# SarthakYadav/leaf-pytorch

Hardware: AMD Instinct MI355X
Metric: LEAF frames/s (40 filt, 16 kHz, 1 s clips) (higher is better)
Workload: dtype f32

## Files before the change

leaf_pytorch_amd/csrc/leaf_fft_wg.hpp:

```cpp
#pragma once
#include <type_traits>
#include "leaf_fft.hpp"
#include "leaf_inst.hpp"
#include "leaf_wg_queue.hpp"

namespace {

constexpr int kWgRingFloat2 = 1032;
constexpr int kWgFwdBins = 1152;
constexpr int kWgRingFwdFloat2 = kWgFwdBins + 8;

typedef float v2f __attribute__((ext_vector_type(2)));
constexpr int kWgScrStride = 68;
constexpr int kWgScrFloats = 32 * kWgScrStride;

__device__ __forceinline__ unsigned lds_addr(const void* p) {
    return (unsigned)(size_t)(__attribute__((address_space(3))) const char*)p;
}
template <int OFF>
__device__ __forceinline__ void lds_rd8(v2f& dst, unsigned addr) {
    asm volatile("ds_read_b64 %0, %1 offset:%2" : "=v"(dst) : "v"(addr), "i"(OFF));
}
template <int N>
__device__ __forceinline__ void lds_wait8(v2f (&a)[8]) {
    asm volatile("s_waitcnt lgkmcnt(%8)"
                 : "+v"(a[0]), "+v"(a[1]), "+v"(a[2]), "+v"(a[3]), "+v"(a[4]), "+v"(a[5]), "+v"(a[6]), "+v"(a[7])
                 : "i"(N));
}
template <typename OffFn, typename Body>
__device__ __forceinline__ void lds_stream32(unsigned addr, OffFn, Body body) {
    v2f buf[2][8];
    auto issue = [&](auto cc) {
        constexpr int c = decltype(cc)::value;
        lds_rd8<OffFn::off(8 * c + 0)>(buf[c & 1][0], addr); lds_rd8<OffFn::off(8 * c + 1)>(buf[c & 1][1], addr);
        lds_rd8<OffFn::off(8 * c + 2)>(buf[c & 1][2], addr); lds_rd8<OffFn::off(8 * c + 3)>(buf[c & 1][3], addr);
        lds_rd8<OffFn::off(8 * c + 4)>(buf[c & 1][4], addr); lds_rd8<OffFn::off(8 * c + 5)>(buf[c & 1][5], addr);
        lds_rd8<OffFn::off(8 * c + 6)>(buf[c & 1][6], addr); lds_rd8<OffFn::off(8 * c + 7)>(buf[c & 1][7], addr);
    };
    issue(std::integral_constant<int, 0>{});
    issue(std::integral_constant<int, 1>{});
    lds_wait8<8>(buf[0]);
#pragma unroll
    for (int j = 0; j < 8; ++j) body(j, buf[0][j]);
    issue(std::integral_constant<int, 2>{});
    lds_wait8<8>(buf[1]);
#pragma unroll
    for (int j = 0; j < 8; ++j) body(8 + j, buf[1][j]);
    issue(std::integral_constant<int, 3>{});
    lds_wait8<8>(buf[0]);
#pragma unroll
    for (int j = 0; j < 8; ++j) body(16 + j, buf[0][j]);
    lds_wait8<0>(buf[1]);
#pragma unroll
    for (int j = 0; j < 8; ++j) body(24 + j, buf[1][j]);
}
struct OffTwl { static constexpr int off(int i) { return 512 * brev5(i); } };
struct OffRow { static constexpr int off(int k) { return 512 * (k & 15); } };

__device__ __forceinline__ void wg_transpose_store(const float (&v)[32], unsigned scr_lds) {
    unsigned keep;
    asm volatile("s_mov_b32 %0, m0\n\ts_mov_b32 m0, %17\n\ts_nop 0\n\t"
                 "ds_write_addtid_b32 %1 offset:0\n\t"
                 "ds_write_addtid_b32 %2 offset:4352\n\t"
                 "ds_write_addtid_b32 %3 offset:2176\n\t"
                 "ds_write_addtid_b32 %4 offset:6528\n\t"
                 "ds_write_addtid_b32 %5 offset:1088\n\t"
                 "ds_write_addtid_b32 %6 offset:5440\n\t"
                 "ds_write_addtid_b32 %7 offset:3264\n\t"
                 "ds_write_addtid_b32 %8 offset:7616\n\t"
                 "ds_write_addtid_b32 %9 offset:544\n\t"
                 "ds_write_addtid_b32 %10 offset:4896\n\t"
                 "ds_write_addtid_b32 %11 offset:2720\n\t"
                 "ds_write_addtid_b32 %12 offset:7072\n\t"
                 "ds_write_addtid_b32 %13 offset:1632\n\t"
                 "ds_write_addtid_b32 %14 offset:5984\n\t"
                 "ds_write_addtid_b32 %15 offset:3808\n\t"
                 "ds_write_addtid_b32 %16 offset:8160\n\t"
                 "s_mov_b32 m0, %0"
                 : "=&s"(keep)
                 : "v"(v[0]), "v"(v[1]), "v"(v[2]), "v"(v[3]), "v"(v[4]), "v"(v[5]), "v"(v[6]), "v"(v[7]), "v"(v[8]), "v"(v[9]), "v"(v[10]), "v"(v[11]), "v"(v[12]), "v"(v[13]), "v"(v[14]), "v"(v[15]), "s"(scr_lds)
                 : "memory");
    asm volatile("s_mov_b32 %0, m0\n\ts_mov_b32 m0, %17\n\ts_nop 0\n\t"
                 "ds_write_addtid_b32 %1 offset:272\n\t"
                 "ds_write_addtid_b32 %2 offset:4624\n\t"
                 "ds_write_addtid_b32 %3 offset:2448\n\t"
                 "ds_write_addtid_b32 %4 offset:6800\n\t"
                 "ds_write_addtid_b32 %5 offset:1360\n\t"
                 "ds_write_addtid_b32 %6 offset:5712\n\t"
                 "ds_write_addtid_b32 %7 offset:3536\n\t"
                 "ds_write_addtid_b32 %8 offset:7888\n\t"
                 "ds_write_addtid_b32 %9 offset:816\n\t"
                 "ds_write_addtid_b32 %10 offset:5168\n\t"
                 "ds_write_addtid_b32 %11 offset:2992\n\t"
                 "ds_write_addtid_b32 %12 offset:7344\n\t"
                 "ds_write_addtid_b32 %13 offset:1904\n\t"
                 "ds_write_addtid_b32 %14 offset:6256\n\t"
                 "ds_write_addtid_b32 %15 offset:4080\n\t"
                 "ds_write_addtid_b32 %16 offset:8432\n\t"
                 "s_mov_b32 m0, %0"
                 : "=&s"(keep)
                 : "v"(v[16]), "v"(v[17]), "v"(v[18]), "v"(v[19]), "v"(v[20]), "v"(v[21]), "v"(v[22]), "v"(v[23]), "v"(v[24]), "v"(v[25]), "v"(v[26]), "v"(v[27]), "v"(v[28]), "v"(v[29]), "v"(v[30]), "v"(v[31]), "s"(scr_lds)
                 : "memory");
}

constexpr int kWgColStride = 36;
constexpr int kWgScrHalfFloats = 32 * kWgColStride;
template <int UPPER>
__device__ __forceinline__ void wg_transpose_store_cols(const float (&v)[32], unsigned scr_lds) {
    unsigned keep;
    unsigned long long save;
    const unsigned base = scr_lds - (UPPER ? 128u : 0u);
    const unsigned long long mask = UPPER ? 0xFFFFFFFF00000000ull : 0x00000000FFFFFFFFull;
    asm volatile("s_mov_b32 %0, m0\n\ts_mov_b64 %1, exec\n\ts_mov_b32 m0, %18\n\ts_mov_b64 exec, %19\n\t"
                 "ds_write_addtid_b32 %2 offset:0\n\t"
                 "ds_write_addtid_b32 %3 offset:2304\n\t"
                 "ds_write_addtid_b32 %4 offset:1152\n\t"
                 "ds_write_addtid_b32 %5 offset:3456\n\t"
                 "ds_write_addtid_b32 %6 offset:576\n\t"
                 "ds_write_addtid_b32 %7 offset:2880\n\t"
                 "ds_write_addtid_b32 %8 offset:1728\n\t"
                 "ds_write_addtid_b32 %9 offset:4032\n\t"
                 "ds_write_addtid_b32 %10 offset:288\n\t"
                 "ds_write_addtid_b32 %11 offset:2592\n\t"
                 "ds_write_addtid_b32 %12 offset:1440\n\t"
                 "ds_write_addtid_b32 %13 offset:3744\n\t"
                 "ds_write_addtid_b32 %14 offset:864\n\t"
                 "ds_write_addtid_b32 %15 offset:3168\n\t"
                 "ds_write_addtid_b32 %16 offset:2016\n\t"
                 "ds_write_addtid_b32 %17 offset:4320\n\t"
                 "s_mov_b64 exec, %1\n\ts_mov_b32 m0, %0"
                 : "=&s"(keep), "=&s"(save)
                 : "v"(v[0]), "v"(v[1]), "v"(v[2]), "v"(v[3]), "v"(v[4]), "v"(v[5]), "v"(v[6]), "v"(v[7]), "v"(v[8]), "v"(v[9]), "v"(v[10]), "v"(v[11]), "v"(v[12]), "v"(v[13]), "v"(v[14]), "v"(v[15]), "s"(base), "s"(mask)
                 : "memory");
    asm volatile("s_mov_b32 %0, m0\n\ts_mov_b64 %1, exec\n\ts_mov_b32 m0, %18\n\ts_mov_b64 exec, %19\n\t"
                 "ds_write_addtid_b32 %2 offset:144\n\t"
                 "ds_write_addtid_b32 %3 offset:2448\n\t"
                 "ds_write_addtid_b32 %4 offset:1296\n\t"
                 "ds_write_addtid_b32 %5 offset:3600\n\t"
                 "ds_write_addtid_b32 %6 offset:720\n\t"
                 "ds_write_addtid_b32 %7 offset:3024\n\t"
                 "ds_write_addtid_b32 %8 offset:1872\n\t"
                 "ds_write_addtid_b32 %9 offset:4176\n\t"
                 "ds_write_addtid_b32 %10 offset:432\n\t"
                 "ds_write_addtid_b32 %11 offset:2736\n\t"
                 "ds_write_addtid_b32 %12 offset:1584\n\t"
                 "ds_write_addtid_b32 %13 offset:3888\n\t"
                 "ds_write_addtid_b32 %14 offset:1008\n\t"
                 "ds_write_addtid_b32 %15 offset:3312\n\t"
                 "ds_write_addtid_b32 %16 offset:2160\n\t"
                 "ds_write_addtid_b32 %17 offset:4464\n\t"
                 "s_mov_b64 exec, %1\n\ts_mov_b32 m0, %0"
                 : "=&s"(keep), "=&s"(save)
                 : "v"(v[16]), "v"(v[17]), "v"(v[18]), "v"(v[19]), "v"(v[20]), "v"(v[21]), "v"(v[22]), "v"(v[23]), "v"(v[24]), "v"(v[25]), "v"(v[26]), "v"(v[27]), "v"(v[28]), "v"(v[29]), "v"(v[30]), "v"(v[31]), "s"(base), "s"(mask)
                 : "memory");
}

__device__ __forceinline__ void fft_build_twiddles_wg(float2* twl, float2* twp, int tid, int nthreads) {
    for (int i = tid; i < 32 * 64; i += nthreads) {
        const int k1 = i >> 6, l = i & 63;
        float s, c;
        sincospif(2.0f * (float)((l * k1) & (kFftN - 1)) / (float)kFftN, &s, &c);
        twl[i] = make_float2(c, -s);
    }
    for (int i = tid; i < 64; i += nthreads) {
        const int h = i >> 5, e = i & 31, j = (e >> 1) + 16 * (e & 1);
        float s, c;
        sincospif(2.0f * (float)j / 64.0f, &s, &c);
        twp[i] = h ? make_float2(c, -s) : make_float2(1.0f, 0.0f);
    }
}
template <int OFF>
__device__ __forceinline__ void lds_rd16(f32x4& dst, unsigned addr) {
    asm volatile("ds_read_b128 %0, %1 offset:%2" : "=v"(dst) : "v"(addr), "i"(OFF));
}
template <int N>
__device__ __forceinline__ void lds_wait16x4(f32x4 (&a)[4]) {
    asm volatile("s_waitcnt lgkmcnt(%4)" : "+v"(a[0]), "+v"(a[1]), "+v"(a[2]), "+v"(a[3]) : "i"(N));
}
template <typename Body>
__device__ __forceinline__ void lds_stream16q(unsigned addr, Body body) {
    f32x4 buf[2][4];
    auto issue = [&](auto cc) {
        constexpr int c = decltype(cc)::value;
        lds_rd16<16 * (4 * c + 0)>(buf[c & 1][0], addr); lds_rd16<16 * (4 * c + 1)>(buf[c & 1][1], addr);
        lds_rd16<16 * (4 * c + 2)>(buf[c & 1][2], addr); lds_rd16<16 * (4 * c + 3)>(buf[c & 1][3], addr);
    };
    issue(std::integral_constant<int, 0>{});
    issue(std::integral_constant<int, 1>{});
    lds_wait16x4<4>(buf[0]);
#pragma unroll
    for (int j = 0; j < 4; ++j) body(j, buf[0][j]);
    issue(std::integral_constant<int, 2>{});
    lds_wait16x4<4>(buf[1]);
#pragma unroll
    for (int j = 0; j < 4; ++j) body(4 + j, buf[1][j]);
    issue(std::integral_constant<int, 3>{});
    lds_wait16x4<4>(buf[0]);
#pragma unroll
    for (int j = 0; j < 4; ++j) body(8 + j, buf[0][j]);
    lds_wait16x4<0>(buf[1]);
#pragma unroll
    for (int j = 0; j < 4; ++j) body(12 + j, buf[1][j]);
}

}
#include "leaf_band.hpp"
namespace {

__device__ __forceinline__ void wg_multiply_stage1(const float2* A, int lane, const float (&rq)[32], float (&zre)[32], float (&zim)[32]) {
    const unsigned a_lo = lds_addr(A + lane), a_hi = lds_addr(A + (kFftN - 64 * 31) - lane);
    v2f lo[16], hi[16];
    auto rd = [&](auto kk) {
        constexpr int k = decltype(kk)::value;
        if constexpr (k < 16) lds_rd8<512 * k>(lo[k], a_lo);
        else lds_rd8<512 * (31 - k)>(hi[k - 16], a_hi);
    };
#define LEAF_RD8(B) rd(std::integral_constant<int, B + 0>{}); rd(std::integral_constant<int, B + 1>{}); \
                    rd(std::integral_constant<int, B + 2>{}); rd(std::integral_constant<int, B + 3>{}); \
                    rd(std::integral_constant<int, B + 4>{}); rd(std::integral_constant<int, B + 5>{}); \
                    rd(std::integral_constant<int, B + 6>{}); rd(std::integral_constant<int, B + 7>{});
    v2f(&lo0)[8] = *reinterpret_cast<v2f(*)[8]>(&lo[0]);
    v2f(&lo1)[8] = *reinterpret_cast<v2f(*)[8]>(&lo[8]);
    v2f(&hi0)[8] = *reinterpret_cast<v2f(*)[8]>(&hi[0]);
    v2f(&hi1)[8] = *reinterpret_cast<v2f(*)[8]>(&hi[8]);
    auto pair = [&](int k) {
        const float ra = rq[k], rb = rq[k + 16];
        const float tr_ = lo[k].x * ra, ti_ = -(lo[k].y * ra);
        zre[k] = fmaf(hi[k].x, rb, tr_);
        zim[k] = fmaf(hi[k].y, rb, ti_);
        zre[k + 16] = fmaf(-hi[k].x, rb, tr_);
        zim[k + 16] = fmaf(-hi[k].y, rb, ti_);
    };
    asm volatile("s_waitcnt lgkmcnt(0)" ::: "memory");
    LEAF_RD8(0) LEAF_RD8(16) LEAF_RD8(8)
    lds_wait8<8>(lo0);
    lds_wait8<8>(hi0);
#pragma unroll
    for (int k = 0; k < 8; ++k) pair(k);
    LEAF_RD8(24)
    lds_wait8<0>(lo1);
    lds_wait8<0>(hi1);
#pragma unroll
    for (int k = 8; k < 16; ++k) pair(k);
#undef LEAF_RD8
}

template <bool HALF, bool SKIP1 = false>
__device__ __forceinline__ void fft2048w(float (&re)[32], float (&im)[32], float* scr, unsigned scr_lds, const float2* twl,
                                         const float2* twh, int lane) {
    if constexpr (SKIP1) {
        fft32_dit_stage<2>(re, im);
        fft32_dit_stage<4>(re, im);
        fft32_dit_stage<8>(re, im);
        fft32_dit_stage<16>(re, im);
    } else {
        fft32_dif(re, im);
    }
    lds_stream32(lds_addr(twl + lane), OffTwl{}, [&](int i, v2f w) {
        if (i == 0) return;
        const float r = re[i] * w.x - im[i] * w.y;
        im[i] = re[i] * w.y + im[i] * w.x;
        re[i] = r;
    });
    const int k1r = lane & 31, h = lane >> 5;
    float tr[32], ti[32];
    const float sg = h ? -1.0f : 1.0f;
    if constexpr (HALF) {
        const f32x4* row = reinterpret_cast<const f32x4*>(scr + k1r * kWgColStride);
        auto plane = [&](const float (&src)[32], float (&t)[32]) {
            f32x4 a[8], b[8];
            wg_transpose_store_cols<0>(src, scr_lds);
#pragma unroll
            for (int q = 0; q < 8; ++q) a[q] = row[q];
            wg_transpose_store_cols<1>(src, scr_lds);
#pragma unroll
            for (int q = 0; q < 8; ++q) b[q] = row[q];
#pragma unroll
            for (int q = 0; q < 8; ++q) {
                t[4 * q] = fmaf(b[q].x, sg, a[q].x); t[4 * q + 1] = fmaf(b[q].y, sg, a[q].y);
                t[4 * q + 2] = fmaf(b[q].z, sg, a[q].z); t[4 * q + 3] = fmaf(b[q].w, sg, a[q].w);
            }
            asm volatile("" ::: "memory");
        };
        pin32(re);
        pin32(im);
        plane(re, tr);
        pin32(tr);
        plane(im, ti);
        pin32(ti);
    } else {
        const f32x4* lo = reinterpret_cast<const f32x4*>(scr + k1r * kWgScrStride);
        auto plane = [&](const float (&src)[32], float (&t)[32]) {
            wg_transpose_store(src, scr_lds);
#pragma unroll
            for (int q0 = 0; q0 < 8; q0 += 4) {
#pragma unroll
                for (int q = q0; q < q0 + 4; ++q) {
                    const f32x4 a = lo[q], b = lo[q + 8];
                    t[4 * q] = fmaf(b.x, sg, a.x); t[4 * q + 1] = fmaf(b.y, sg, a.y);
                    t[4 * q + 2] = fmaf(b.z, sg, a.z); t[4 * q + 3] = fmaf(b.w, sg, a.w);
                }
                asm volatile("" ::: "memory");
            }
        };
        pin32(re);
        pin32(im);
        plane(re, tr);
        pin32(tr);
        plane(im, ti);
        pin32(ti);
    }
    lds_stream16q(lds_addr(twh + 32 * h), [&](int j, f32x4 w) {
        float ar, ai;
        if (j == 0) {
            ar = tr[0];
            ai = ti[0];
        } else {
            ar = tr[j] * w.x - ti[j] * w.y;
            ai = tr[j] * w.y + ti[j] * w.x;
        }
        const float br = tr[j + 16], bi = ti[j + 16];
        const float pr = fmaf(-bi, w.w, fmaf(br, w.z, ar));
        const float pi = fmaf(bi, w.z, fmaf(br, w.w, ai));
        re[j] = pr;
        im[j] = pi;
        re[j + 16] = fmaf(2.0f, ar, -pr);
        im[j + 16] = fmaf(2.0f, ai, -pi);
    });
    fft32_dit_stage<2>(re, im);
    fft32_dit_stage<4>(re, im);
    fft32_dit_stage<8>(re, im);
    fft32_dit_stage<16>(re, im);
}

constexpr int fft_wg_scr_floats(int NW) { return NW > 12 ? kWgScrHalfFloats : kWgScrFloats; }
constexpr size_t fft_wg_lds_bytes(int NW, int SK) {
    return ((size_t)kTwFloats + 2 * 2 * kWgRingFwdFloat2 + kWgQueueInts +
            (size_t)NW * fft_wg_scr_floats(NW)) * 4;
}
constexpr int wg_gcd(int a, int b) { return b == 0 ? a : wg_gcd(b, a % b); }
constexpr int wg_pool_step(int SHOP) { return wg_gcd(64, SHOP); }
constexpr int wg_pool_jmin(int SK, int SHOP) {
    const int g = wg_pool_step(SHOP), padl = SK / 2 + SK % 2 - 1;
    return -63 + (((padl + 63) % g) + g) % g;
}
constexpr int wg_pool_nj(int SK, int SHOP) { return (SK - 1 - wg_pool_jmin(SK, SHOP)) / wg_pool_step(SHOP) + 1; }

constexpr int wg_pow2_ceil(int v) { int r = 1; while (r < v) r <<= 1; return r; }
constexpr int kWgStreamMaxLag = 6;
constexpr int wg_stream_lag(int SK, int SHOP, int ring) {
    const int padl = SK / 2 + SK % 2 - 1, ls = fft_block_len(SK, SHOP, true);
    const int dmax = (ls - 1 + padl) / SHOP, mf = (ls - SK + padl) / SHOP, fb = ls / SHOP;
    const int lag = ((ring + mf - dmax) / fb) & ~1;
    return lag > kWgStreamMaxLag ? kWgStreamMaxLag : lag;
}
constexpr int wg_stream_ring_min(int SK, int SHOP) {
    int r = 8;
    while (wg_stream_lag(SK, SHOP, r) < 2) r <<= 1;
    return r;
}
constexpr int wg_stream_fp(int F) { return F | 1; }
constexpr int kWgOutChunk = 32;
constexpr int kWgOutRow = 2 * kWgOutChunk + 1;
constexpr size_t fft_wg_stream_lds_bytes(int NW, int SK, int ring, int F) {
    return fft_wg_lds_bytes(NW, SK) + ((size_t)ring * wg_stream_fp(F) + wg_stream_fp(F) + 8 * (size_t)F + 8 +
                                       (size_t)F * kWgOutRow) * 4;
}

constexpr int kWgXF32 = 0, kWgX16 = 1, kWgXMix = 2, kWgXMix16 = 3;
constexpr int kWgXAny = 4;
template <int SK, int SHOP, int XK>
__device__ __forceinline__ void wg_load_block(const FftParams& p, int gb, int lane, float (&are)[32], int& b, int& c) {
    constexpr int PADL = SK / 2 + SK % 2 - 1;
    constexpr int LS = fft_block_len(SK, SHOP, true);
    constexpr bool ANY = XK == kWgXAny;
    b = gb / p.nblk;
    c = gb - b * p.nblk;
    const int n_c = c * LS;
    const float* xb = static_cast<const float*>(p.x) + (size_t)b * p.T;
    const unsigned short* xh = static_cast<const unsigned short*>(p.x) + (size_t)b * p.T;
    if (ANY ? p.mix_lam != nullptr : (XK == kWgXMix || XK == kWgXMix16)) {
        const MixClip mc = mix_clip(p.mix_perm, p.mix_lam, b, p.B, p.T);
        const size_t row = (size_t)b * p.T;
        if constexpr (ANY) {
            const int st = p.io_bf16 == kSamplePcm16 ? kSamplePcm16 : kSampleF32;
#pragma unroll
            for (int r = 0; r < 32; ++r) {
                const int i = 64 * r + lane;
                const int n = n_c - PADL + ((i + PADL) & (kFftN - 1));
                const float w = mix_load(p.x, row, mc.partner, (size_t)min(max(n, 0), p.T - 1), mc.lam, mc.om, st);
                are[r] = (n >= 0 && n < p.T) ? w : 0.0f;
            }
        } else if (XK == kWgXMix16) {
#pragma unroll
            for (int r = 0; r < 32; ++r) {
                const int i = 64 * r + lane;
                are[r] = mix_sample<kSamplePcm16>(p.x, row, mc, n_c - PADL + ((i + PADL) & (kFftN - 1)), p.T);
            }
        } else {
#pragma unroll
            for (int r = 0; r < 32; ++r) {
                const int i = 64 * r + lane;
                are[r] = mix_sample<kSampleF32>(p.x, row, mc, n_c - PADL + ((i + PADL) & (kFftN - 1)), p.T);
            }
        }
    } else if (ANY ? p.io_bf16 != 0 : XK == kWgX16) {
        const bool pcm = p.io_bf16 == kSamplePcm16;
#pragma unroll
        for (int r = 0; r < 32; ++r) {
            const int i = 64 * r + lane;
            const int n = n_c - PADL + ((i + PADL) & (kFftN - 1));
            const unsigned v = xh[min(max(n, 0), p.T - 1)];
            const float w = pcm ? pcm16_widen((short)v) : __uint_as_float(v << 16);
            are[r] = (n >= 0 && n < p.T) ? w : 0.0f;
        }
    } else {
#pragma unroll
        for (int r = 0; r < 32; ++r) {
            const int i = 64 * r + lane;
            const int n = n_c - PADL + ((i + PADL) & (kFftN - 1));
            are[r] = (n >= 0 && n < p.T) ? xb[n] : 0.0f;
        }
    }
}

constexpr int kWgTailRows = 4, kWgTailGroup = 16;
constexpr int wg_tail_stride(int CH) { return CH + kWgTailGroup; }
constexpr int wg_tail_floats(int CH) { return 2 * kWgTailRows * wg_tail_stride(CH); }
template <int NW, int CH>
__device__ __forceinline__ void wg_tail_rows(const FinParams& q, int b_lo, int b_hi, float* scr, int wave, int lane) {
    static_assert(CH == 64 || CH == 128, "chunk lengths of the tail");
    constexpr int RB = kWgTailRows, GF = kWgTailGroup, S = wg_tail_stride(CH);
    float* P = scr;
    float* Mt = scr + RB * S;
    const int TP = q.TP, mode = q.mode;
    const SlotGeom geo = q.geo;
    const bool scaled = q.clip_scale2 != nullptr, pcen = (mode & 1) != 0;
    auto ld = [](const float* a) { return __hip_atomic_load(a, __ATOMIC_RELAXED, __HIP_MEMORY_SCOPE_AGENT); };
    auto wave_fence = [] { __builtin_amdgcn_fence(__ATOMIC_ACQ_REL, "wavefront"); };
    const int nrows_all = (b_hi - b_lo) * q.F;
    if (nrows_all <= 0) return;
    const int per = nrows_all / NW, rem = nrows_all - per * NW;
    const int my0 = b_lo * q.F + wave * per + min(wave, rem), mycnt = per + (wave < rem ? 1 : 0);
    for (int r0 = 0; r0 < mycnt; r0 += RB) {
        const int row0 = my0 + r0, nr = min(RB, mycnt - r0);
        const int rl = min(lane >> 4, nr - 1), jl = lane & (GF - 1);
        const int rowl = row0 + rl, bl = rowl / q.F, fl = rowl - bl * q.F;
        const FinCoef c = q.lds_coef ? static_cast<const FinCoef*>(q.lds_coef)[fl] : fin_coef(q, fl);
        const float s2l = scaled ? q.clip_scale2[bl] : 1.0f;
        const bool mine = (lane >> 4) < nr;
        const int re = min(lane, nr - 1);
        FinCoef ce{};
        ce.w = __shfl(c.w, GF * re);
        ce.omw = __shfl(c.omw, GF * re);
        const bool fast = pcen && __all(c.dl > 0.0f);
        const float* prow = P + re * S;
        float* mrow = Mt + re * S;
        auto ema_group = [&](int g, float M) {
            float pv[GF];
#pragma unroll
            for (int k = 0; k < GF; ++k) pv[k] = prow[g * GF + k];
#pragma unroll
            for (int k = 0; k < GF; ++k) {
                M = fin_ema_step(ce, pv[k], M);
                mrow[g * GF + k] = M;
            }
            return M;
        };
        float carry = 0.0f;
        for (int m0 = 0; m0 < TP; m0 += CH) {
            const int nfr = min(CH, TP - m0);
            wave_fence();
            for (int j0 = 0; j0 < nfr; j0 += 64) {
                const bool on = j0 + lane < nfr;
                const int j = min(j0 + lane, nfr - 1), m = m0 + j;
                float a[RB], b2[RB], c3[RB];
                int ns = 1;
                if (q.lds_sums) {
#pragma unroll
                    for (int r = 0; r < RB; ++r) {
                        a[r] = q.lds_sums[(size_t)(row0 + min(r, nr - 1) - q.lds_row0) * TP + m];
                        b2[r] = c3[r] = 0.0f;
                    }
                } else {
                    ns = fin_slots(geo, m);
#pragma unroll
                    for (int r = 0; r < RB; ++r) {
                        const float* pr = q.part + (size_t)(row0 + min(r, nr - 1)) * geo.nslot * TP + m;
                        a[r] = ld(pr);
                        b2[r] = ld(pr + (ns > 1 ? TP : 0));
                        c3[r] = geo.nslot > 2 ? ld(pr + (ns > 2 ? 2 * TP : 0)) : 0.0f;
                    }
                }
#pragma unroll
                for (int r = 0; r < RB; ++r) {
                    const float bias = __int_as_float(__builtin_amdgcn_readlane(__float_as_int(c.bias), GF * r));
                    const float s2 = __int_as_float(__builtin_amdgcn_readlane(__float_as_int(s2l), GF * r));
                    float v = fin_pooled(a[r], b2[r], c3[r], ns, scaled, s2, bias);
                    if (on && r < nr) {
                        if (q.raw_out) q.raw_out[(size_t)(row0 + r) * TP + m] = v;
                        if (!(mode & 8)) v = pooled_floor(v);
                        P[r * S + j] = v;
                    }
                }
            }
            wave_fence();
            const int ng = (nfr + GF - 1) / GF;
            const size_t orow = (size_t)rowl * TP + m0;
            if (fast) {
                float M = ema_group(0, m0 == 0 ? prow[0] : carry);
                for (int g = 0; g < ng; ++g) {
                    wave_fence();
                    const int j = g * GF + jl;
                    const float pv = P[rl * S + j], mv = Mt[rl * S + j];
                    if (g + 1 < ng) M = ema_group(g + 1, M);
                    const float o = fin_point_pcen_pos(c, q.floor_, pv, mv);
                    if (mine && j < nfr) fin_store(q, orow + j, o);
                }
                carry = M;
            } else {
                if (pcen) {
                    float M = m0 == 0 ? prow[0] : carry;
#pragma nounroll
                    for (int j = 0; j < nfr; ++j) {
                        M = fin_ema_step(ce, prow[j], M);
                        mrow[j] = M;
                    }
                    carry = M;
                    wave_fence();
                }
#pragma nounroll
                for (int g = 0; g < ng; ++g) {
                    const int j = g * GF + jl;
                    const float o = fin_point(c, mode, q.floor_, P[rl * S + j], pcen ? Mt[rl * S + j] : 0.0f);
                    if (mine && j < nfr) fin_store(q, orow + j, o);
                }
            }
        }
    }
}

template <int SK, int SHOP, int NW, bool STREAM, int XK, int TAILC>
__device__ __forceinline__ void leaf_fft_wg_body(const FftParams& p) {
    constexpr bool HALF = NW > 12;
    constexpr int SCRF = fft_wg_scr_floats(NW);
    extern __shared__ __attribute__((aligned(16))) float wsm[];
    float2* twl = reinterpret_cast<float2*>(wsm);
    float2* twh = twl + 32 * 64;
    float2* ring = twh + 64;
    int* q = reinterpret_cast<int*>(ring + 2 * kWgRingFwdFloat2);
    const int tid = threadIdx.x;
    const int wave = __builtin_amdgcn_readfirstlane(tid >> 6), lane0 = tid & 63;
#if LEAF_TRACE
    const unsigned long long tr_entry = __builtin_amdgcn_s_memtime();
    const unsigned long long tr_entry_rt = __builtin_amdgcn_s_memrealtime();
#endif
    float* scr = reinterpret_cast<float*>(q + kWgQueueInts) + (size_t)wave * SCRF;
    const int RING = p.stream_ring;
    const int FPS = wg_stream_fp(p.F);
    float* fr = reinterpret_cast<float*>(q + kWgQueueInts) + (size_t)NW * SCRF;
    float* ema_st = fr + (size_t)RING * FPS;
    FinCoef* coefT = reinterpret_cast<FinCoef*>(ema_st + FPS);
    static_assert(sizeof(FinCoef) == 32, "8 floats per filter");
    int* sq = reinterpret_cast<int*>(coefT + p.F);
    float* ost = reinterpret_cast<float*>(sq + 8);
    (void)fr; (void)ema_st; (void)coefT; (void)sq; (void)ost;
    float* lsum = reinterpret_cast<float*>(q + kWgQueueInts) + (size_t)NW * SCRF;
    const bool lds_sums = !STREAM && p.fin_fused == 3;
    const unsigned scr_lds = __builtin_amdgcn_readfirstlane(
        (unsigned)(size_t)(__attribute__((address_space(3))) float*)scr);
    constexpr bool BANDK = !HALF && band_geometry_ok(SK, SHOP);
    const bool band_on = BANDK && p.band.rec != nullptr;
    int* bl = reinterpret_cast<int*>(wsm + p.band.lds_off);
    (void)bl;
    if constexpr (BANDK) {
        if (band_on && wave == 0) band_build_plan(p.band.rec, p.band.elist, p.band.n_edge, p.F, bl, lane0, p.band.bias, p.band.smax);
    }

    const bool spec_pre = p.spec0 != nullptr && !HALF && p.B * p.nblk > 0;
    float2 sv[kWgFwdBins / 64];
    if (spec_pre && wave == 1) {
        const float2* src = p.spec0 + (size_t)blockIdx.x * kWgRingFwdFloat2;
#pragma unroll
        for (int k = 0; k < kWgFwdBins / 64; ++k) sv[k] = src[64 * k + lane0];
    }
    constexpr bool EARLYK = !HALF && !STREAM;
    const bool early = EARLYK && p.spec0 == nullptr;
    const int eset = NW - 1 - wave;
    bool early_me = false;
    float ex[32];
    int eb = 0, ec = 0;
    if constexpr (EARLYK) {
        const OwnedClips deal0{p.B * p.nblk, (int)gridDim.x, p.nblk};
        early_me = early && eset < 2 && eset < deal0.count((int)blockIdx.x);
        if (early_me) wg_load_block<SK, SHOP, XK>(p, deal0.start((int)blockIdx.x) + eset, lane0, ex, eb, ec);
    }
    if (BANDK && band_on) { if (wave > 0) fft_build_twiddles_wg(twl, twh, tid - 64, (NW - 1) * 64); }
    else fft_build_twiddles_wg(twl, twh, tid, NW * 64);
    if (tid < kWgQueueInts) q[tid] = (tid == 0 && spec_pre) ? 1 : (tid == 0 && early) ? 2 : 0;
    if constexpr (STREAM) {
        for (int f = tid; f < p.F; f += NW * 64) coefT[f] = fin_coef(p.fin, f);
        if (tid < 8) sq[tid] = 0;
        for (int i = tid; i < RING * FPS; i += NW * 64) fr[i] = 0.0f;
    }
    FinCoef* lcoef = nullptr;
    if (lds_sums) {
        const int n = (int)((long long)p.B * p.nblk / (int)gridDim.x / p.nblk) * p.F * p.TP;
        for (int i = tid; i < n; i += NW * 64) lsum[i] = 0.0f;
        lcoef = reinterpret_cast<FinCoef*>(lsum + (n + 7) / 8 * 8);
        constexpr int NC = NW > 2 ? (NW - 2) * 64 : NW * 64;
        if (tid < NC)
            for (int f = NC - 1 - tid; f < p.F; f += NC) lcoef[f] = fin_coef(p.fin, f);
    }
    __syncthreads();
#if LEAF_TRACE
    int tr_n = 0;
#define WG_STAMP(tag)                                                                                           \
    do {                                                                                                        \
        if (LEAF_TRACE == 2 && (tag) != 1 && (tag) != 2 && (tag) < 8) break;    \
        if (blockIdx.x == 0 && wave < 16 && lane0 == 0 && tr_n < 56)                                            \
            p.trace[wave * 64 + tr_n] = ((unsigned long long)(tag) << 56) | (__builtin_amdgcn_s_memtime() & 0x00FFFFFFFFFFFFFFull); \
        ++tr_n;                                                                                                 \
    } while (0)
#define WG_STAMP_AT(slot, tag, when)                                                                            \
    do {                                                                                                        \
        if (blockIdx.x == 0 && wave < 16 && lane0 == 0)                                                         \
            p.trace[wave * 64 + (slot)] = ((unsigned long long)(tag) << 56) | ((when) & 0x00FFFFFFFFFFFFFFull); \
    } while (0)
#define WG_STAMP_NOW(slot, tag) WG_STAMP_AT(slot, tag, __builtin_amdgcn_s_memtime())
    WG_STAMP_NOW(57, 15);
    WG_STAMP_AT(56, 14, tr_entry);
    WG_STAMP_AT(62, 20, tr_entry_rt);
#else
#define WG_STAMP(tag) do { } while (0)
#define WG_STAMP_AT(slot, tag, when) do { } while (0)
#define WG_STAMP_NOW(slot, tag) do { } while (0)
#endif

    constexpr int PADL = SK / 2 + SK % 2 - 1;
    constexpr int LS = fft_block_len(SK, SHOP, true);
    constexpr int DMIN = -((SK - 1 - PADL) / SHOP);
    constexpr int DMAX = (LS - 1 + PADL) / SHOP;
    constexpr int NFR = DMAX - DMIN + 1;
    constexpr int NROW = LS / 64;
    constexpr int NGRP = (NFR + 15) / 16;
    static_assert(LS % SHOP == 0 && LS % 64 == 0 && LS > 0 && NFR <= 32 && (SK & 1), "static odd-window geometry");
    static_assert(!STREAM || (LS + SK - PADL) / SHOP + 2 <= kWgOutChunk, "a block completes fewer frames than one output chunk");

    const OwnedClips deal{p.B * p.nblk, (int)gridDim.x, p.nblk};
    if (spec_pre && wave == 1) {
        const int gb0 = deal.start((int)blockIdx.x);
#pragma unroll
        for (int k = 0; k < kWgFwdBins / 64; ++k) ring[64 * k + lane0] = sv[k];
        wg_publish(q, 0, gb0 / p.nblk, gb0 % p.nblk, lane0);
        WG_STAMP_NOW(58, 16);
    }
    if (early_me) {
        WG_STAMP(1);
        float eim[32];
#pragma unroll
        for (int r = 0; r < 32; ++r) eim[r] = 0.0f;
        fft2048w<HALF>(ex, eim, scr, scr_lds, twl, twh, lane0);
        float2* A = ring + eset * kWgRingFwdFloat2;
#pragma unroll
        for (int i = 0; i < 32; ++i) {
            const int k = brev5(i);
            if (k < kWgFwdBins / 64) A[64 * k + lane0] = make_float2(ex[i], eim[i]);
        }
        wg_publish(q, eset, eb, ec, lane0);
        if (eset == 0) WG_STAMP_NOW(58, 16);
    }
    const int first_gb = deal.start((int)blockIdx.x);
    const int nset = deal.count((int)blockIdx.x);
    const int NT = band_on ? __builtin_amdgcn_readfirstlane(bl[0]) : p.F;
    const int* tdesc = bl + kBandPlanHead;
    const int* bmem = tdesc + p.F + 4;
    (void)tdesc; (void)bmem;
    const WgTaskCursor cur = wg_task_cursor(q, lane0, NT, nset);
    auto desc_of = [&](int role) {
        if (role <= 0 || role > NT) return 0;
        return band_on ? __builtin_amdgcn_readfirstlane(tdesc[role - 1]) : (role - 1) << 2;
    };
    float rq[32];
    auto prefetch_task = [&](int role, int lane) {
        const int d = desc_of(role);
        if constexpr (BANDK) {
            if ((d & 3) == 1) { band_load_spectrum<16>(rq, reinterpret_cast<const float*>(p.H), bmem[(d >> 2) + lane / band_lpf(16)], lane); return; }
            if ((d & 3) == 2) { band_load_spectrum<32>(rq, reinterpret_cast<const float*>(p.H), bmem[(d >> 2) + lane / band_lpf(32)], lane); return; }
        }
        wg_load_real_spectrum(rq, p.H, d >> 2, lane);
    };

    auto stream_finalize = [&](int j) {
        WG_STAMP(10);
        if (j > 0) wg_wait_ge(wgq_stream_out_cnt(q, (j - 1) & 1), ((j - 1) >> 1) + 1);
        WG_STAMP(8);
        __builtin_amdgcn_s_setprio(3);
        const int gb = first_gb + j;
        const int b = gb / p.nblk, c = gb - b * p.nblk;
        const int gbase = ((gb - first_gb) / p.nblk) * p.TP;
        const int mf_prev = c == 0 ? -1 : min(p.TP - 1, (c * LS - SK + PADL) / SHOP);
        const int mf = c == p.nblk - 1 ? p.TP - 1 : min(p.TP - 1, ((c + 1) * LS - SK + PADL) / SHOP);
        const int mode = p.fin.mode;
        const bool scaled = p.fin.clip_scale2 != nullptr;
        const float s2 = scaled ? p.fin.clip_scale2[b] : 1.0f;
#ifndef LEAF_STREAM_ABLATE
#define LEAF_STREAM_ABLATE 0
#endif
        constexpr int G = 4;
        for (int f0 = 0; f0 < p.F && LEAF_STREAM_ABLATE != 1; f0 += 64) {
            const int f = f0 + lane0;
            const bool on = f < p.F;
            const FinCoef cf = coefT[on ? f : 0];
            const bool fast = __all(!on || cf.dl > 0.0f);
            float M = (c == 0 || !on) ? 0.0f : ema_st[f];
            const size_t orow = ((size_t)b * p.F + (on ? f : 0)) * p.TP;
            for (int base = mf_prev + 1; base <= mf; base += G) {
                const int cnt = min(G, mf - base + 1);
                float sa[G], sb[G], v[G], Mv[G];
                int ns[G];
#pragma unroll
                for (int k = 0; k < G; ++k) {
                    const int m = min(base + k, mf);
                    float* e = fr + (size_t)((gbase + m) & (RING - 1)) * FPS + (on ? f : 0);
                    ns[k] = 1;
                    sa[k] = e[0];
                    sb[k] = 0.0f;
                    if (on && k < cnt) e[0] = 0.0f;
                }
#pragma unroll
                for (int k = 0; k < G; ++k) {
                    const int m = base + k;
                    float x = fin_pooled(sa[k], sb[k], 0.0f, ns[k], scaled, s2, cf.bias);
                    if (k < cnt && on && p.fin.raw_out) p.fin.raw_out[orow + m] = x;
                    if (!(mode & 8)) x = pooled_floor(x);
                    v[k] = x;
                    if ((mode & 1) && k < cnt) {
                        if (m == 0) M = x;
                        M = fin_ema_step(cf, x, M);
                    }
                    Mv[k] = M;
                }
                if (fast && (mode & 1)) {
                    float o[G];
#pragma unroll
                    for (int k = 0; k < G; ++k) o[k] = fin_point_pcen_pos(cf, p.fin.floor_, v[k], Mv[k]);
#pragma unroll
                    for (int k = 0; k < G; ++k)
                        if (k < cnt && on && (LEAF_STREAM_ABLATE != 2 || o[k] == 12345.678f))
                            ost[f * kWgOutRow + ((base + k) & (2 * kWgOutChunk - 1))] = o[k];
                } else {
#pragma unroll
                    for (int k = 0; k < G; ++k) {
                        const float ov = fin_point_outofline(cf, mode, p.fin.floor_, v[k], Mv[k]);
                        if (k < cnt && on) ost[f * kWgOutRow + ((base + k) & (2 * kWgOutChunk - 1))] = ov;
                    }
                }
            }
            if (on) ema_st[f] = M;
        }
        if (LEAF_STREAM_ABLATE != 1) {
            const int q0 = (mf_prev + 1) / kWgOutChunk;
            const int q1 = c == p.nblk - 1 ? (p.TP - 1) / kWgOutChunk : (mf + 1) / kWgOutChunk - 1;
            for (int qc = q0; qc <= q1; ++qc) {
                const int m = qc * kWgOutChunk + (lane0 & (kWgOutChunk - 1));
                for (int r0 = 0; r0 < p.F; r0 += 64 / kWgOutChunk) {
                    const int row = r0 + lane0 / kWgOutChunk;
                    if (row < p.F && m < p.TP)
                        fin_store(p.fin, ((size_t)b * p.F + row) * p.TP + m, ost[row * kWgOutRow + (m & (2 * kWgOutChunk - 1))]);
                }
            }
        }
        __builtin_amdgcn_s_setprio(0);
        WG_STAMP(9);
        wg_release();
        wg_bump(wgq_stream_out_cnt(q, j & 1), lane0);
    };
    (void)stream_finalize;

    int seen_set = -1, seen_b = 0, seen_c = 0, seen_base = 0, seen_clip = 0;
    int set = 0, role = 0;
    int t = cur.next(set, role);
    prefetch_task(role, lane0);
    while (cur.has(t)) {
        int lane = lane0;
        asm volatile("" : "+v"(lane));
        const int slot = set & 1, gen = set >> 1;
        float2* A = ring + slot * kWgRingFwdFloat2;
        WG_STAMP(role == 0 ? 1 : 2);
        if (role == 0) {
            if (set < nset) {
                float are[32], aim[32];
                int fb, fc;
                wg_load_block<SK, SHOP, XK>(p, first_gb + set, lane, are, fb, fc);
#pragma unroll
                for (int r = 0; r < 32; ++r) aim[r] = 0.0f;
                fft2048w<HALF>(are, aim, scr, scr_lds, twl, twh, lane);
                wg_wait_ge(wgq_readers_cnt(q, slot), gen * NT);
                if constexpr (STREAM) {
                    const int lag = wg_stream_lag(SK, SHOP, RING);
                    if (set >= lag) wg_wait_ge(wgq_stream_out_cnt(q, slot), gen - lag / 2 + 1);
                }
#pragma unroll
                for (int i = 0; i < 32; ++i) {
                    const int k = brev5(i);
                    if (k < kWgFwdBins / 64) A[64 * k + lane] = make_float2(are[i], aim[i]);
                }
                wg_publish(q, slot, fb, fc, lane);
                if (set == 0) WG_STAMP_NOW(58, 16);
            }
            t = cur.next(set, role);
            prefetch_task(role, lane);
            continue;
        }
        const int tdsc = desc_of(role);
        const int f = tdsc >> 2;
        if (set != seen_set) {
            wg_acquire_block(q, slot, gen, seen_b, seen_c);
            if constexpr (STREAM) seen_base = ((set - seen_c) / p.nblk) * p.TP;
            seen_clip = lds_sums ? (set - seen_c) / p.nblk : 0;
            seen_set = set;
        }
        WG_STAMP(3);
        const int b = seen_b, c = seen_c;
        const int n_c = c * LS;
        const int Lv = min(LS, p.T - n_c);
        int mlo = n_c + PADL - SK + 1;
        mlo = mlo <= 0 ? 0 : (mlo + SHOP - 1) / SHOP;
        const int mhi = min(p.TP - 1, (n_c + Lv - 1 + PADL) / SHOP);
        if constexpr (BANDK) {
            if (tdsc & 3) {
                int tn_b = 0, nset_b = 0, nrole_b = 0;
                auto mid = [&]() {
                    tn_b = cur.next(nset_b, nrole_b);
                    prefetch_task(nrole_b, lane);
                    return std::integral_constant<int, 32>{};
                };
                auto stamp = [&](int tag) { (void)tag; WG_STAMP(tag); };
                auto bout = [&](int fid, int m, float v) {
                    const int first_block = max(0, m * SHOP - PADL) / LS;
                    if constexpr (STREAM)
                        __hip_atomic_fetch_add(&fr[(size_t)((seen_base + m) & (RING - 1)) * FPS + fid], v, __ATOMIC_RELAXED, __HIP_MEMORY_SCOPE_WORKGROUP);
                    else if (lds_sums)
                        __hip_atomic_fetch_add(&lsum[((size_t)seen_clip * p.F + fid) * p.TP + m], v, __ATOMIC_RELAXED, __HIP_MEMORY_SCOPE_WORKGROUP);
                    else
                        p.part[(((size_t)b * p.F + fid) * p.nslot + (c - first_block)) * p.TP + m] = v;
                };
                if ((tdsc & 3) == 1)
                    band_task<16, SK, SHOP>(p, rq, A, bmem + (tdsc >> 2), bl + 4, twl, scr, scr_lds, q, slot, c, mlo, mhi, lane, mid, bout, stamp);
                else
                    band_task<32, SK, SHOP>(p, rq, A, bmem + (tdsc >> 2), bl + 4, twl, scr, scr_lds, q, slot, c, mlo, mhi, lane, mid, bout, stamp);
                if constexpr (STREAM) {
                    const int done = wg_count(&sq[set & 7], lane);
                    if (done + 1 == ((set >> 3) + 1) * NT) stream_finalize(set);
                }
                WG_STAMP(7);
                t = tn_b;
                set = nset_b;
                role = nrole_b;
                continue;
            }
        }
        float zre[32], zim[32];
        {
            const unsigned a_lo = lds_addr(A + lane), a_hi = lds_addr(A + (kFftN - 64 * 31) - lane);
            v2f lo[16], hi[16];
            auto rd = [&](auto kk) {
                constexpr int k = decltype(kk)::value;
                if constexpr (k < 16) lds_rd8<512 * k>(lo[k], a_lo);
                else lds_rd8<512 * (31 - k)>(hi[k - 16], a_hi);
            };
            (void)rd;
#define LEAF_RD8(B) rd(std::integral_constant<int, B + 0>{}); rd(std::integral_constant<int, B + 1>{}); \
                    rd(std::integral_constant<int, B + 2>{}); rd(std::integral_constant<int, B + 3>{}); \
                    rd(std::integral_constant<int, B + 4>{}); rd(std::integral_constant<int, B + 5>{}); \
                    rd(std::integral_constant<int, B + 6>{}); rd(std::integral_constant<int, B + 7>{});
            v2f(&lo0)[8] = *reinterpret_cast<v2f(*)[8]>(&lo[0]);
            v2f(&lo1)[8] = *reinterpret_cast<v2f(*)[8]>(&lo[8]);
            v2f(&hi0)[8] = *reinterpret_cast<v2f(*)[8]>(&hi[0]);
            v2f(&hi1)[8] = *reinterpret_cast<v2f(*)[8]>(&hi[8]);
            auto pair = [&](int k) {
                const float ra = rq[k], rb = rq[k + 16];
                const float tr_ = lo[k].x * ra, ti_ = -(lo[k].y * ra);
                zre[k] = fmaf(hi[k].x, rb, tr_);
                zim[k] = fmaf(hi[k].y, rb, ti_);
                zre[k + 16] = fmaf(-hi[k].x, rb, tr_);
                zim[k + 16] = fmaf(-hi[k].y, rb, ti_);
            };
            LEAF_RD8(0) LEAF_RD8(16) LEAF_RD8(8)
            lds_wait8<8>(lo0);
            lds_wait8<8>(hi0);
#pragma unroll
            for (int k = 0; k < 8; ++k) pair(k);
            LEAF_RD8(24)
            lds_wait8<0>(lo1);
            lds_wait8<0>(hi1);
#pragma unroll
            for (int k = 8; k < 16; ++k) pair(k);
#undef LEAF_RD8
        }
        asm volatile("s_waitcnt lgkmcnt(0)" ::"v"(zre[31]), "v"(zim[31]) : "memory");
        wg_reader_done(q, slot, lane);
        WG_STAMP(4);
        fft2048w<HALF, true>(zre, zim, scr, scr_lds, twl, twh, lane);
        WG_STAMP(5);
        constexpr int PG = wg_pool_step(SHOP), PJ0 = wg_pool_jmin(SK, SHOP), NJ = wg_pool_nj(SK, SHOP);
        float pw[NJ];
        {
            const float* gsrc = p.Gz + (size_t)f * p.GZ + (kGPad + PJ0) + lane;
            asm volatile("" ::: "memory");
#pragma unroll
            for (int k = 0; k < NJ; ++k) pw[k] = gsrc[PG * k];
            asm volatile("" ::: "memory");
        }
        float er[NROW];
#pragma unroll
        for (int i = 0; i < 32; ++i) {
            const int r = brev5(i);
            if (r < NROW) er[r] = zre[i] * zre[i] + zim[i] * zim[i];
        }
        if (Lv < LS) {
#pragma unroll
            for (int r = 0; r < NROW; ++r) er[r] = 64 * r + lane < Lv ? er[r] : 0.0f;
        }
        int nset_i = 0, nrole = 0;
        const int tn = cur.next(nset_i, nrole);
        asm volatile("" ::"v"(er[0]), "v"(er[NROW - 1]));
        prefetch_task(nrole, lane);
        asm volatile("s_waitcnt vmcnt(32)" ::: "memory");
        WG_STAMP(6);
        float acc[NGRP][16];
#pragma unroll
        for (int g = 0; g < NGRP; ++g)
#pragma unroll
            for (int fi = 0; fi < 16; ++fi) acc[g][fi] = 0.0f;
#pragma unroll
        for (int r = 0; r < NROW; ++r) {
#pragma unroll
            for (int fi = 0; fi < NFR; ++fi) {
                const int is = (DMIN + fi) * SHOP - PADL;
                if (is <= 64 * r + 63 && is + SK > 64 * r) {
                    static_assert((PADL - PJ0) % PG == 0, "window offsets are congruent to padL modulo gcd(64, hop)");
                    acc[fi / 16][fi % 16] = fmaf(er[r], pw[(64 * r - is - PJ0) / PG], acc[fi / 16][fi % 16]);
                }
            }
        }
        asm volatile("" : "+v"(acc[0][0]));
#pragma unroll
        for (int g = 0; g < NGRP; ++g) {
            const float v = frame_butterfly16(acc[g], lane);
            const int fi = 16 * g + ((lane >> 5) & 1) * 8 + ((lane >> 4) & 1) * 4 + ((lane >> 3) & 1) * 2 + ((lane >> 2) & 1);
            const int m = n_c / SHOP + DMIN + fi;
            if ((lane & 3) == 0 && fi < NFR && m >= mlo && m <= mhi) {
                const int first_block = max(0, m * SHOP - PADL) / LS;
                if constexpr (STREAM)
                    __hip_atomic_fetch_add(&fr[(size_t)((seen_base + m) & (RING - 1)) * FPS + f], v, __ATOMIC_RELAXED, __HIP_MEMORY_SCOPE_WORKGROUP);
                else if (lds_sums)
                    __hip_atomic_fetch_add(&lsum[((size_t)seen_clip * p.F + f) * p.TP + m], v, __ATOMIC_RELAXED, __HIP_MEMORY_SCOPE_WORKGROUP);
                else
                    p.part[(((size_t)b * p.F + f) * p.nslot + (c - first_block)) * p.TP + m] = v;
            }
        }
        if constexpr (STREAM) {
            const int done = wg_count(&sq[set & 7], lane);
            if (done + 1 == ((set >> 3) + 1) * NT) stream_finalize(set);
        }
        WG_STAMP(7);
        t = tn;
        set = nset_i;
        role = nrole;
    }
    WG_STAMP_NOW(59, 17);
    if constexpr (!STREAM) {
        if (p.fin_fused) {
            const int b_lo = (first_gb + p.nblk - 1) / p.nblk, b_hi = (first_gb + nset) / p.nblk;
            static_assert(SCRF >= wg_tail_floats(TAILC), "a wave's transposition scratch holds its rows of a chunk");
            FinParams fin = p.fin;
            if (lds_sums) {
                fin.lds_sums = lsum;
                fin.lds_row0 = b_lo * p.F;
                fin.lds_coef = lcoef;
            }
            __builtin_amdgcn_fence(__ATOMIC_RELEASE, "workgroup");
            __syncthreads();
            WG_STAMP_NOW(60, 18);
            wg_tail_rows<NW, TAILC>(fin, b_lo, b_hi, scr, wave, lane0);
            WG_STAMP_NOW(61, 19);
            WG_STAMP_AT(63, 21, __builtin_amdgcn_s_memrealtime());
        }
    }
}

template <int SK, int SHOP, int NW, bool STREAM = false>
__global__ __launch_bounds__(NW * 64, (NW + 3) / 4) void leaf_fft_wg_kernel(const FftParams p) {
    leaf_fft_wg_body<SK, SHOP, NW, STREAM, STREAM ? kWgXAny : kWgXF32, STREAM ? 0 : 128>(p);
}
template <int SK, int SHOP, int NW, int XK, int TAILC>
__global__ __launch_bounds__(NW * 64, (NW + 3) / 4) void leaf_fft_wg_kernel_var(const FftParams p) {
    static_assert(XK != kWgXAny && (XK != kWgXF32 || TAILC != 128) && (TAILC == 64 || TAILC == 128), "that pair is leaf_fft_wg_kernel");
    leaf_fft_wg_body<SK, SHOP, NW, false, XK, TAILC>(p);
}
template <int SK, int SHOP, int NW, int XK, int TAILC>
constexpr FftKernel wg_tail_kernel() {
    if constexpr (XK == kWgXF32 && TAILC == 128) return leaf_fft_wg_kernel<SK, SHOP, NW, false>;
    else return leaf_fft_wg_kernel_var<SK, SHOP, NW, XK, TAILC>;
}
template <int XK, int TAILC>
inline FftKernel wg_tail_instance_of(int sk, int nw) {
    if (sk == 401 && nw == 12) return wg_tail_kernel<401, 160, 12, XK, TAILC>();
    if (sk == 801 && nw == 10) return wg_tail_kernel<801, 320, 10, XK, TAILC>();
    if (sk == 201 && nw == 12) return wg_tail_kernel<201, 80, 12, XK, TAILC>();
    return nullptr;
}
template <int XK>
inline FftKernel wg_tail_instance(int sk, int nw, int tailc) {
    return tailc == 128 ? wg_tail_instance_of<XK, 128>(sk, nw) : tailc == 64 ? wg_tail_instance_of<XK, 64>(sk, nw) : nullptr;
}

}
```

Measured before the change: 311.9 million.

## Rebalance fused finalize tail into wave-wide row batches with 6-frame groups

The fused PCEN/finalize tail now packs up to 10 rows per wave batch, using 6-lane groups and 60-frame chunks, instead of 4 rows with 16-lane groups and 64/128-frame chunks. Rows are split into batches that are spread evenly across waves, and the per-row source offsets are hoisted out of the chunk loop. The aim is to fill all 64 lanes and shorten the serial EMA chain per group so the tail after the FFT finishes sooner. The costs are more chunk iterations, a non-power-of-two lane split that needs integer division, and the TAILC template parameter no longer being used by the tail.

```diff
diff --git a/leaf_pytorch_amd/csrc/leaf_fft_wg.hpp b/leaf_pytorch_amd/csrc/leaf_fft_wg.hpp
--- a/leaf_pytorch_amd/csrc/leaf_fft_wg.hpp
+++ b/leaf_pytorch_amd/csrc/leaf_fft_wg.hpp
@@ -424,13 +424,13 @@
     }
 }
 
-constexpr int kWgTailRows = 4, kWgTailGroup = 16;
-constexpr int wg_tail_stride(int CH) { return CH + kWgTailGroup; }
-constexpr int wg_tail_floats(int CH) { return 2 * kWgTailRows * wg_tail_stride(CH); }
-template <int NW, int CH>
-__device__ __forceinline__ void wg_tail_rows(const FinParams& q, int b_lo, int b_hi, float* scr, int wave, int lane) {
-    static_assert(CH == 64 || CH == 128, "chunk lengths of the tail");
-    constexpr int RB = kWgTailRows, GF = kWgTailGroup, S = wg_tail_stride(CH);
+constexpr int kWgTailGroup = 6, kWgTailChunk = 60, kWgTailStride = 70;
+constexpr int wg_tail_rows_max(int scrf) { return 2 * 10 * kWgTailStride <= scrf ? 10 : 8; }
+constexpr int wg_tail_floats(int rows) { return 2 * rows * kWgTailStride; }
+template <int NW, int RB>
+__device__ __forceinline__ bool wg_tail_rows(const FinParams& q, int b_lo, int b_hi, float* scr, int wave, int lane) {
+    constexpr int GF = kWgTailGroup, CH = kWgTailChunk, S = kWgTailStride;
+    static_assert(RB * GF <= 64 && CH % GF == 0 && CH <= 64 && 64 <= S && S % 32 == GF, "a batch is one wave wide; a chunk is one pass");
     float* P = scr;
     float* Mt = scr + RB * S;
     const int TP = q.TP, mode = q.mode;
@@ -439,16 +439,16 @@
     auto ld = [](const float* a) { return __hip_atomic_load(a, __ATOMIC_RELAXED, __HIP_MEMORY_SCOPE_AGENT); };
     auto wave_fence = [] { __builtin_amdgcn_fence(__ATOMIC_ACQ_REL, "wavefront"); };
     const int nrows_all = (b_hi - b_lo) * q.F;
-    if (nrows_all <= 0) return;
-    const int per = nrows_all / NW, rem = nrows_all - per * NW;
-    const int my0 = b_lo * q.F + wave * per + min(wave, rem), mycnt = per + (wave < rem ? 1 : 0);
-    for (int r0 = 0; r0 < mycnt; r0 += RB) {
-        const int row0 = my0 + r0, nr = min(RB, mycnt - r0);
-        const int rl = min(lane >> 4, nr - 1), jl = lane & (GF - 1);
+    const int nb = (nrows_all + RB - 1) / RB;
+    if (wave >= nb) return false;
+    const int per = nrows_all / nb, rem = nrows_all - per * nb;
+    for (int bi = wave; bi < nb; bi += NW) {
+        const int row0 = b_lo * q.F + bi * per + min(bi, rem), nr = per + (bi < rem ? 1 : 0);
+        const int rl = min(lane / GF, nr - 1), jl = lane - (lane / GF) * GF;
         const int rowl = row0 + rl, bl = rowl / q.F, fl = rowl - bl * q.F;
         const FinCoef c = q.lds_coef ? static_cast<const FinCoef*>(q.lds_coef)[fl] : fin_coef(q, fl);
         const float s2l = scaled ? q.clip_scale2[bl] : 1.0f;
-        const bool mine = (lane >> 4) < nr;
+        const bool mine = lane / GF < nr;
         const int re = min(lane, nr - 1);
         FinCoef ce{};
         ce.w = __shfl(c.w, GF * re);
@@ -456,6 +456,12 @@
         const bool fast = pcen && __all(c.dl > 0.0f);
         const float* prow = P + re * S;
         float* mrow = Mt + re * S;
+        const int rstride = q.lds_sums ? TP : geo.nslot * TP;
+        const float* src = q.lds_sums ? q.lds_sums + (size_t)(row0 - q.lds_row0) * TP : q.part + (size_t)row0 * geo.nslot * TP;
+        float* raw = q.raw_out ? q.raw_out + (size_t)row0 * TP : nullptr;
+        int roff[RB];
+#pragma unroll
+        for (int r = 0; r < RB; ++r) roff[r] = min(r, nr - 1) * rstride;
         auto ema_group = [&](int g, float M) {
             float pv[GF];
 #pragma unroll
@@ -471,38 +477,41 @@
         for (int m0 = 0; m0 < TP; m0 += CH) {
             const int nfr = min(CH, TP - m0);
             wave_fence();
-            for (int j0 = 0; j0 < nfr; j0 += 64) {
-                const bool on = j0 + lane < nfr;
-                const int j = min(j0 + lane, nfr - 1), m = m0 + j;
-                float a[RB], b2[RB], c3[RB];
-                int ns = 1;
+            {
+                const bool on = lane < nfr;
+                const int j = min(lane, nfr - 1), m = m0 + j;
+                float v[RB];
+                auto pooled = [&](int r, float a, float b2, float c3, int ns) {
+                    const float bias = __int_as_float(__builtin_amdgcn_readlane(__float_as_int(c.bias), GF * r));
+                    const float s2 = __int_as_float(__builtin_amdgcn_readlane(__float_as_int(s2l), GF * r));
+                    v[r] = fin_pooled(a, b2, c3, ns, scaled, s2, bias);
+                };
                 if (q.lds_sums) {
+                    float a[RB];
+#pragma unroll
+                    for (int r = 0; r < RB; ++r) a[r] = src[roff[r] + m];
+#pragma unroll
+                    for (int r = 0; r < RB; ++r) pooled(r, a[r], 0.0f, 0.0f, 1);
+                } else {
+                    float a[RB], b2[RB], c3[RB];
+                    const int ns = fin_slots(geo, m);
 #pragma unroll
                     for (int r = 0; r < RB; ++r) {
-                        a[r] = q.lds_sums[(size_t)(row0 + min(r, nr - 1) - q.lds_row0) * TP + m];
-                        b2[r] = c3[r] = 0.0f;
-                    }
-                } else {
-                    ns = fin_slots(geo, m);
-#pragma unroll
-                    for (int r = 0; r < RB; ++r) {
-                        const float* pr = q.part + (size_t)(row0 + min(r, nr - 1)) * geo.nslot * TP + m;
+                        const float* pr = src + roff[r] + m;
                         a[r] = ld(pr);
                         b2[r] = ld(pr + (ns > 1 ? TP : 0));
                         c3[r] = geo.nslot > 2 ? ld(pr + (ns > 2 ? 2 * TP : 0)) : 0.0f;
                     }
-                }
-#pragma unroll
-                for (int r = 0; r < RB; ++r) {
-                    const float bias = __int_as_float(__builtin_amdgcn_readlane(__float_as_int(c.bias), GF * r));
-                    const float s2 = __int_as_float(__builtin_amdgcn_readlane(__float_as_int(s2l), GF * r));
-                    float v = fin_pooled(a[r], b2[r], c3[r], ns, scaled, s2, bias);
-                    if (on && r < nr) {
-                        if (q.raw_out) q.raw_out[(size_t)(row0 + r) * TP + m] = v;
-                        if (!(mode & 8)) v = pooled_floor(v);
-                        P[r * S + j] = v;
-                    }
-                }
+#pragma unroll
+                    for (int r = 0; r < RB; ++r) pooled(r, a[r], b2[r], c3[r], ns);
+                }
+                if (q.raw_out) {
+#pragma unroll
+                    for (int r = 0; r < RB; ++r)
+                        if (on && r < nr) raw[r * TP + m] = v[r];
+                }
+#pragma unroll
+                for (int r = 0; r < RB; ++r) P[r * S + lane] = (mode & 8) ? v[r] : pooled_floor(v[r]);
             }
             wave_fence();
             const int ng = (nfr + GF - 1) / GF;
@@ -538,6 +547,7 @@
             }
         }
     }
+    return true;
 }
 
 template <int SK, int SHOP, int NW, bool STREAM, int XK, int TAILC>
@@ -974,7 +984,8 @@
     if constexpr (!STREAM) {
         if (p.fin_fused) {
             const int b_lo = (first_gb + p.nblk - 1) / p.nblk, b_hi = (first_gb + nset) / p.nblk;
-            static_assert(SCRF >= wg_tail_floats(TAILC), "a wave's transposition scratch holds its rows of a chunk");
+            constexpr int TAILR = wg_tail_rows_max(SCRF);
+            static_assert(SCRF >= wg_tail_floats(TAILR), "a wave's transposition scratch holds its rows of a chunk");
             FinParams fin = p.fin;
             if (lds_sums) {
                 fin.lds_sums = lsum;
@@ -984,9 +995,15 @@
             __builtin_amdgcn_fence(__ATOMIC_RELEASE, "workgroup");
             __syncthreads();
             WG_STAMP_NOW(60, 18);
-            wg_tail_rows<NW, TAILC>(fin, b_lo, b_hi, scr, wave, lane0);
-            WG_STAMP_NOW(61, 19);
-            WG_STAMP_AT(63, 21, __builtin_amdgcn_s_memrealtime());
+            [[maybe_unused]] const bool tailed = wg_tail_rows<NW, TAILR>(fin, b_lo, b_hi, scr, wave, lane0);
+#if LEAF_TRACE
+            if (tailed) {
+                unsigned hw_id;
+                asm volatile("s_getreg_b32 %0, hwreg(HW_REG_HW_ID)" : "=s"(hw_id));
+                WG_STAMP_NOW(61, 19 | ((hw_id >> 4) & 3) << 5);
+                WG_STAMP_AT(63, 21, __builtin_amdgcn_s_memrealtime());
+            }
+#endif
         }
     }
 }
```

New measurement: 308.1 million. 0.988x the previous value.
